# david-cortes/MatrixExtra

Hardware: AMD Instinct MI355X
Metric: CSR x dense SpMM GFLOP/s (fp64, 1M x 100k, 32 nnz/row, k=128) + achieved HBM BW% vs CPU ref (higher is better)
Workload: dtype f64; 1 GPU; dgRMatrix 1000000x100000 nnz/row=32 f64 %*% dense 100000x128 (BASELINE configs[1]); C col-major; rows_per_gpu=1000000, cols=100000, nnz_per_row=32, dense_cols=128, parallelism=single

## Files before the change

### matrixextra_amd/csrc/spmm_common.h

```cpp
#pragma once
#include "mx_dispatch.h"

struct mx_spmm_plan {
    int m = 0, K = 0, npanels = 0, panel_cols = 0, noct = 0;
    long long total_steps = 0;
    long long nnz = 0;
    int32_t *step_off = nullptr; size_t step_off_cap = 0;
    int32_t *pcol = nullptr;     size_t pcol_cap = 0;
    double *pval = nullptr;      size_t pval_cap = 0;
    void *scratch = nullptr;     size_t scratch_cap = 0;
    bool ready = false;
    bool pending = false;
    const int32_t *indptr = nullptr, *indices = nullptr;
    const double *values = nullptr;
    const int32_t *oct_off = nullptr;
    const long long *sizes = nullptr;
    int *go = nullptr;
    long long fill_cap = 0;
    int pad_rule = 0;
};

namespace mx {

template <typename T, int N> struct VecT;
template <> struct VecT<double, 1> { using type = double; };
template <> struct VecT<double, 2> { using type = double __attribute__((ext_vector_type(2))); };
template <> struct VecT<float, 1>  { using type = float; };
template <> struct VecT<float, 2>  { using type = float __attribute__((ext_vector_type(2))); };
template <> struct VecT<float, 4>  { using type = float __attribute__((ext_vector_type(4))); };

template <typename real_t, int VEC>
__device__ __forceinline__ void vload(real_t (&dst)[VEC], const real_t *__restrict__ p)
{
    using V = typename VecT<real_t, VEC>::type;
    if constexpr (VEC == 1) {
        dst[0] = *p;
    } else {
        const V v = *reinterpret_cast<const V *>(p);
#pragma unroll
        for (int i = 0; i < VEC; i++) dst[i] = v[i];
    }
}

template <typename real_t, int VEC>
__device__ __forceinline__ void vstore(real_t *__restrict__ p, const real_t (&src)[VEC])
{
    using V = typename VecT<real_t, VEC>::type;
    if constexpr (VEC == 1) {
        *p = src[0];
    } else {
        V v;
#pragma unroll
        for (int i = 0; i < VEC; i++) v[i] = src[i];
        *reinterpret_cast<V *>(p) = v;
    }
}

template <typename real_t, int VEC>
__device__ __forceinline__ void vstore_nt(real_t *__restrict__ p, const real_t (&src)[VEC])
{
    using V = typename VecT<real_t, VEC>::type;
    if constexpr (VEC == 1) {
        __builtin_nontemporal_store(src[0], p);
    } else {
        V v;
#pragma unroll
        for (int i = 0; i < VEC; i++) v[i] = src[i];
        __builtin_nontemporal_store(v, reinterpret_cast<V *>(p));
    }
}

__device__ __forceinline__ double mx_fma(double a, double b, double c) { return __builtin_fma(a, b, c); }
__device__ __forceinline__ float mx_fma(float a, float b, float c) { return __builtin_fmaf(a, b, c); }

constexpr int SLAB_GROUP = 8;
template <typename real_t> constexpr int SLAB_VEC = 16 / (int)sizeof(real_t);
template <typename real_t> constexpr int SLAB_W = SLAB_GROUP * SLAB_VEC<real_t>;

__device__ __forceinline__ void xcd_timing_barrier(unsigned *ctr, unsigned target)
{
    __syncthreads();
    if (threadIdx.x == 0) {
        __hip_atomic_fetch_add(ctr, 1u, __ATOMIC_RELAXED, __HIP_MEMORY_SCOPE_AGENT);
        int spins = 0;
        while (__hip_atomic_load(ctr, __ATOMIC_RELAXED, __HIP_MEMORY_SCOPE_AGENT) < target && ++spins < 4096)
            __builtin_amdgcn_s_sleep(8);
    }
    __syncthreads();
}

inline int pick_panels(int K, size_t l2_budget)
{
    const size_t slab_bytes = (size_t)K * 128;
    int p = (int)((slab_bytes + l2_budget - 1) / l2_budget);
    if (p < 1) p = 1;
    if (p > 64) p = 64;
    return p;
}

template <typename real_t>
inline bool slab_ok(int n, const real_t *B, size_t ldb, const real_t *C, size_t ldc, int colmajor)
{
    constexpr int VEC = SLAB_VEC<real_t>;
    if (n < VEC || n % VEC || ldb % VEC || (uintptr_t)B % 16) return false;
    if (!colmajor && (ldc % VEC || (uintptr_t)C % 16)) return false;
    return true;
}

#pragma GCC visibility push(hidden)
void kt_begin(hipStream_t st);
void kt_end(hipStream_t st);
void note_spmm_kernel(const char *name);
unsigned persistent_grid(int wg_per_cu, long long total_items);
constexpr size_t SYNC_BYTES = 8 * 64 * sizeof(unsigned);
void *pack_workspace(size_t bytes);
unsigned *sync_workspace();

template <typename real_t>
int launch_repack(int K, int Kp, int n, const real_t *B, size_t ldb, real_t *Bp, const int *go, hipStream_t st);
int launch_spmm_slab(int m, int n, int K, const int32_t *indptr, const int32_t *indices, const double *values,
                     const void *B, size_t ldb, void *C, size_t ldc, int dense_dtype, int colmajor, int npanels,
                     int wg_per_cu, hipStream_t stream);

int plan_begin(mx_spmm_plan *pl, int m, int K, const int32_t *indptr, const int32_t *indices, const double *values,
               int npanels, hipStream_t st, int pad_rule = 0);
int plan_end(mx_spmm_plan *pl, hipStream_t st, bool *refilled = nullptr);
int plan_repack(int K, int n, const void *B, size_t ldb, int dense_dtype, hipStream_t st, void **Bp_out,
                const int *go = nullptr);
int plan_run(const mx_spmm_plan *pl, int n, const void *B, size_t ldb, void *C, size_t ldc, int dense_dtype,
             int colmajor, int wg_per_cu, int sync_mode, hipStream_t st, const void *Bp = nullptr);
#pragma GCC visibility pop

}
```

### matrixextra_amd/csrc/spmm_plan.hip

```cpp
#include "spmm_common.h"
#include <new>

namespace mx {

constexpr int PLAN_RB = 8;
constexpr int PLAN_OCT_ROWS = PLAN_RB * 8;
constexpr int PLAN_MAXP = 64;
constexpr int PLAN_DEFAULT_WG_PER_CU = 1;
constexpr int PLAN_CHUNK = 4;
constexpr int PLAN_TAIL_SLOTS = 512;
constexpr int PLAN_ROW_SHIFT = 27;

constexpr int PLAN_LD = 4;
constexpr int PLAN_STAGE_STEPS = 384;
constexpr int PLAN_PAD_NUM = 7, PLAN_PAD_DEN = 4;

__host__ __device__ __forceinline__ bool plan_accept(long long total, long long nnz, long long cap_slots, int pad_rule)
{
    if (total < 0 || total * 8 + PLAN_TAIL_SLOTS > cap_slots) return false;
    return !(pad_rule && total * 8 * PLAN_PAD_DEN > nnz * PLAN_PAD_NUM + 65536LL * PLAN_PAD_DEN);
}

__device__ __forceinline__ int panel_of(int col, int panel_cols, float inv_pc, int npanels)
{
    int q = (int)((float)col * inv_pc);
    const int r = col - q * panel_cols;
    q += r >= panel_cols ? 1 : (r < 0 ? -1 : 0);
    return q < npanels ? q : npanels - 1;
}

__global__ __launch_bounds__(256)
void plan_size_kernel(int m, int noct, const int32_t *__restrict__ indptr, int32_t *__restrict__ steps,
                      long long *__restrict__ nnz_out)
{
    const int b = blockIdx.x * 256 + threadIdx.x;
    if (b == 0) *nnz_out = indptr[m];
    int len = 0;
    if (b < noct * 8) {
        const int r0 = min(b * PLAN_RB, m), r1 = min(b * PLAN_RB + PLAN_RB, m);
        len = indptr[r1] - indptr[r0];
    }
    len = max(len, __shfl_xor(len, 1, 8));
    len = max(len, __shfl_xor(len, 2, 8));
    len = max(len, __shfl_xor(len, 4, 8));
    if (b < noct * 8 && (b & 7) == 0)
        steps[b >> 3] = (len + 8 * PLAN_CHUNK - 1) & ~(8 * PLAN_CHUNK - 1);
}

__device__ __forceinline__ unsigned long long multisplit_peers(int key, const unsigned long long (&bal)[6], int nbits,
                                                                unsigned long long valid)
{
    unsigned long long peers = valid;
#pragma unroll
    for (int b = 0; b < 6; b++)
        if (b < nbits) peers &= ((key >> b) & 1) ? bal[b] : ~bal[b];
    return peers;
}

__global__ __launch_bounds__(512, 8)
void plan_fill_kernel(int m, int npanels, int panel_cols, const int32_t *__restrict__ indptr,
                      const int32_t *__restrict__ indices, const double *__restrict__ values,
                      const int32_t *__restrict__ oct_off, int32_t *__restrict__ pcol, double *__restrict__ pval,
                      int noct, int pad_col, int32_t *__restrict__ step_off,
                      const long long *__restrict__ sizes, long long cap_slots, int pad_rule, int *__restrict__ go)
{
    __shared__ int32_t s_col[PLAN_STAGE_STEPS * 8];
    __shared__ double s_val[PLAN_STAGE_STEPS * 8];
    __shared__ int s_bpo[8][PLAN_MAXP];

    const bool ok = plan_accept(sizes[0], sizes[1], cap_slots, pad_rule);
    if (blockIdx.x == 0 && threadIdx.x == 0) *go = ok ? 1 : 0;
    if (!ok) return;

    const int g = threadIdx.x >> 6, lane = threadIdx.x & 63;
    const int oct = blockIdx.x;
    const int row0 = oct * PLAN_OCT_ROWS + g * PLAN_RB;
    int rp[PLAN_RB + 1];
#pragma unroll
    for (int r = 0; r <= PLAN_RB; r++) rp[r] = uniform(indptr[min(row0 + r, m)]);
    const int s = rp[0], e = rp[PLAN_RB];
    const int base = oct_off[oct];
    const int steps_oct = oct_off[oct + 1] - base;
    const bool stage = steps_oct <= PLAN_STAGE_STEPS;
    const float inv_pc = 1.0f / (float)panel_cols;
    const int nbits = npanels > 1 ? 32 - __clz(npanels - 1) : 0;
    const unsigned long long below = (1ULL << lane) - 1ULL;

    int col0[PLAN_LD];
    double val0[PLAN_LD];
#pragma unroll
    for (int c = 0; c < PLAN_LD; c++) {
        const int k = s + 64 * c + lane;
        col0[c] = -1; val0[c] = 0.0;
        if (k < e) { col0[c] = indices[k]; val0[c] = values[k]; }
    }
    auto split = [&](int pan, unsigned long long (&bal)[6]) -> unsigned long long {
#pragma unroll
        for (int b = 0; b < 6; b++)
            bal[b] = b < nbits ? __ballot(pan >= 0 && ((pan >> b) & 1)) : 0ULL;
        return __ballot(pan >= 0);
    };

    int mine = 0;
    for (int k0 = s; k0 < e; k0 += 64 * PLAN_LD) {
        int colv[PLAN_LD];
#pragma unroll
        for (int c = 0; c < PLAN_LD; c++) {
            const int k = k0 + 64 * c + lane;
            colv[c] = col0[c];
            if (k0 != s) colv[c] = k < e ? indices[k] : -1;
        }
#pragma unroll
        for (int c = 0; c < PLAN_LD; c++) {
            if (k0 + 64 * c >= e) break;
            const int pan = colv[c] >= 0 ? panel_of(colv[c], panel_cols, inv_pc, npanels) : -1;
            unsigned long long bal[6];
            const unsigned long long valid = split(pan, bal);
            if (lane < npanels) mine += __popcll(multisplit_peers(lane, bal, nbits, valid));
        }
    }
    int incl = lane < npanels ? mine : 0;
#pragma unroll
    for (int off = 1; off < 64; off <<= 1) {
        const int up = __shfl_up(incl, off, 64);
        if (lane >= off) incl += up;
    }
    int nextstep = incl - mine;
    s_bpo[g][lane] = nextstep;

    auto put = [&](int t, int word, double v) {
        const int slot = (t & ~7) * 8 + g * 8 + (t & 7);
        if (stage) { s_col[slot] = word; s_val[slot] = v; }
        else { pcol[(size_t)base * 8 + slot] = word; pval[(size_t)base * 8 + slot] = v; }
    };

    for (int k0 = s; k0 < e; k0 += 64 * PLAN_LD) {
        int colv[PLAN_LD];
        double av[PLAN_LD];
#pragma unroll
        for (int c = 0; c < PLAN_LD; c++) {
            const int k = k0 + 64 * c + lane;
            colv[c] = col0[c]; av[c] = val0[c];
            if (k0 != s) {
                colv[c] = -1; av[c] = 0.0;
                if (k < e) { colv[c] = indices[k]; av[c] = values[k]; }
            }
        }
#pragma unroll
        for (int c = 0; c < PLAN_LD; c++) {
            if (k0 + 64 * c >= e) break;
            const int k = k0 + 64 * c + lane;
            const int col = colv[c];
            int pan = -1, lrow = 0;
            if (col >= 0) {
                pan = panel_of(col, panel_cols, inv_pc, npanels);
#pragma unroll
                for (int r = 1; r < PLAN_RB; r++) lrow += k >= rp[r];
            }
            unsigned long long bal[6];
            const unsigned long long valid = split(pan, bal);
            const int start = __shfl(nextstep, pan < 0 ? 0 : pan, 64);
            if (pan >= 0) put(start + __popcll(multisplit_peers(pan, bal, nbits, valid) & below), col | (lrow << PLAN_ROW_SHIFT), av[c]);
            if (lane < npanels) nextstep += __popcll(multisplit_peers(lane, bal, nbits, valid));
        }
    }
    int last_lrow = 0;
    if (e > s) {
#pragma unroll
        for (int r = 1; r < PLAN_RB; r++) last_lrow += (e - 1) >= rp[r];
    }
    for (int t = (e - s) + lane; t < steps_oct; t += 64) put(t, pad_col | (last_lrow << PLAN_ROW_SHIFT), 0.0);

    __syncthreads();
    if (g == 0 && lane < npanels) {
        int sum = 0;
#pragma unroll
        for (int gg = 0; gg < 8; gg++) sum += s_bpo[gg][lane];
        step_off[(size_t)oct * npanels + lane] = base + (lane == 0 ? 0 : sum / 8);
        if (oct == noct - 1 && lane == 0) step_off[(size_t)noct * npanels] = oct_off[noct];
    }
    if (stage) {
        const int nslots = steps_oct * 8;
        int4 *gc = reinterpret_cast<int4 *>(pcol + (size_t)base * 8);
        const int4 *lc = reinterpret_cast<const int4 *>(s_col);
        for (int i = threadIdx.x; i < nslots / 4; i += 512) gc[i] = lc[i];
        using d2 = double __attribute__((ext_vector_type(2)));
        d2 *gv = reinterpret_cast<d2 *>(pval + (size_t)base * 8);
        const d2 *lv = reinterpret_cast<const d2 *>(s_val);
        for (int i = threadIdx.x; i < nslots / 2; i += 512) gv[i] = lv[i];
    }
    if (oct == noct - 1) {
        static_assert(PLAN_TAIL_SLOTS == 512, "one slot per thread of the last block");
        const size_t dst = (size_t)oct_off[noct] * 8 + threadIdx.x;
        pcol[dst] = pad_col;
        pval[dst] = 0.0;
    }
}

template <int U>
__device__ __forceinline__ int group8_dpp_bcast(int v)
{
    int t = __builtin_amdgcn_mov_dpp(v, 0x150 + U, 0xF, 0x3, false);
    return __builtin_amdgcn_update_dpp(t, v, 0x150 + 8 + U, 0xF, 0xC, false);
}
template <int U>
__device__ __forceinline__ void plan_bcast(int pcw, double pvw, int &pc, double &pv)
{
    union { double d; int i[2]; } a, b;
    a.d = pvw;
    pc = group8_dpp_bcast<U>(pcw);
    b.i[0] = group8_dpp_bcast<U>(a.i[0]);
    b.i[1] = group8_dpp_bcast<U>(a.i[1]);
    pv = b.d;
}

template <int VEC>
__device__ __forceinline__ void lds_fold(double *d, double (&acc)[VEC])
{
#pragma unroll
    for (int v = 0; v < VEC; v++) __hip_atomic_fetch_add(d + v, acc[v], __ATOMIC_RELAXED, __HIP_MEMORY_SCOPE_WORKGROUP);
}
template <int VEC>
__device__ __forceinline__ void lds_fold(float *d, float (&acc)[VEC])
{
#pragma unroll
    for (int v = 0; v < VEC; v++) d[v] += acc[v];
}

#ifdef MX_SWEEP_PROBE
__device__ unsigned long long g_sweep_probe[8][8];
#define MX_PROBE(...) __VA_ARGS__
#else
#define MX_PROBE(...)
#endif

template <typename real_t, bool COLMAJOR, int PLAN_WAVES>
__global__ __launch_bounds__(PLAN_WAVES * 64)
void spmm_plan_kernel(int m, int n, int npanels, const int32_t *__restrict__ step_off,
                      const int32_t *__restrict__ pcol, const double *__restrict__ pval,
                      const real_t *__restrict__ Bp, size_t slab_stride,
                      real_t *__restrict__ C, size_t ldc, int nslabs, int ngens, int noct, int pad_col,
                      unsigned *__restrict__ sync_ctr, int sync_mode)
{
    constexpr int VEC = 16 / (int)sizeof(real_t);
    constexpr int W = SLAB_GROUP * VEC;
    constexpr int U = 8;
    constexpr int PLAN_WG_ROWS = PLAN_OCT_ROWS * PLAN_WAVES;
    constexpr int S = W + 16 / (int)sizeof(real_t) / 2;
    __shared__ real_t accs[PLAN_WG_ROWS * S];

    const int lane = threadIdx.x & 63, wave = threadIdx.x >> 6, g = lane >> 3, lg = lane & 7;
    const int xcd = blockIdx.x & 7, wg = blockIdx.x >> 3, nwg = gridDim.x >> 3;
    const long long total = (long long)nslabs * ngens;
    const long long lo = total * xcd / 8, hi = total * (xcd + 1) / 8;
    const int niter = (int)((hi - lo + nwg - 1) / nwg);
    unsigned *const my_ctr = sync_ctr + xcd * 64;
    real_t *const my_oct = accs + (size_t)wave * PLAN_OCT_ROWS * S;
    real_t *const my_rows = my_oct + (size_t)g * PLAN_RB * S + lg * VEC;
    MX_PROBE(long long pr_t = 0; int pr_kind = 0; unsigned long long pr_sum[3] = {0, 0, 0}; unsigned pr_cnt[3] = {0, 0, 0};)

    for (int it = 0; it < niter; it++) {
        const long long item_raw = lo + wg + (long long)it * nwg;
        const bool have = item_raw < hi;
        const long long item = have ? item_raw : lo;
        const int slab = (int)(item / ngens), gen = (int)(item % ngens);
        const int oct = gen * PLAN_WAVES + wave;
        const bool oct_ok = have && oct < noct;
        const char *__restrict__ Bbase = reinterpret_cast<const char *>(Bp + (size_t)slab * slab_stride);
        const unsigned lane_off = (unsigned)(lg * VEC * sizeof(real_t));

        for (int i = lane; i < PLAN_OCT_ROWS * S; i += 64) my_oct[i] = 0;
        if (sync_mode > 0) __syncthreads();

        {
            if (sync_mode >= 2) xcd_timing_barrier(my_ctr, (unsigned)(it + 1) * (unsigned)nwg);
            int so_row = 0, so_end = 0;
            if (oct_ok) {
                if (lane < npanels) so_row = step_off[(size_t)oct * npanels + lane];
                so_end = step_off[(size_t)oct * npanels + npanels];
            }
            const int sbeg = __builtin_amdgcn_readfirstlane(so_row);
            const int send = __builtin_amdgcn_readfirstlane(so_end);
            int next_b = npanels > 1 ? __builtin_amdgcn_readlane(so_row, 1) : send;
            int p = 0;
            int cur = 0;
            real_t acc[VEC];
#pragma unroll
            for (int v = 0; v < VEC; v++) acc[v] = 0;
            static_assert(U == 8, "one batch = one wavefront of plan slots");
            static_assert(W * sizeof(real_t) == 128, "slab line");
            auto b_offset = [&](int c) -> unsigned {
                return ((unsigned)c * (unsigned)(W * sizeof(real_t))) + lane_off;
            };
            int rc[PLAN_CHUNK], rn[PLAN_CHUNK];
            double rv[PLAN_CHUNK], rvn[PLAN_CHUNK];
            auto load_chunk = [&](int step, int (&c)[PLAN_CHUNK], double (&v)[PLAN_CHUNK]) {
                const long long e = (long long)step * 8 + lane;
#pragma unroll
                for (int k = 0; k < PLAN_CHUNK; k++) { c[k] = pcol[e + 64 * k]; v[k] = pval[e + 64 * k]; }
            };
            int pc[U];
            double pv[U];
            real_t b[U][VEC];
#pragma unroll
            for (int u = 0; u < U; u++) {
                pc[u] = 0;
                pv[u] = 0.0;
#pragma unroll
                for (int v = 0; v < VEC; v++) b[u][v] = 0;
            }
            auto consume = [&](int u) {
                const int lrow = (int)((unsigned)pc[u] >> PLAN_ROW_SHIFT);
                if (lrow != cur) {
                    lds_fold<VEC>(my_rows + cur * S, acc);
#pragma unroll
                    for (int v = 0; v < VEC; v++) acc[v] = 0;
                    cur = lrow;
                }
                const real_t a = (real_t)pv[u];
#pragma unroll
                for (int v = 0; v < VEC; v++) acc[v] = mx_fma(a, b[u][v], acc[v]);
#pragma unroll
                for (int v = 0; v < VEC; v++) asm volatile("" : "+v"(acc[v]));
                __builtin_amdgcn_sched_barrier(0);
            };
            if (send > sbeg) {
                load_chunk(sbeg, rc, rv);
#pragma unroll
                for (int k = 0; k < PLAN_CHUNK; k++) asm volatile("" : "+v"(rc[k]), "+v"(rv[k]));
            }
            for (int s = sbeg; s < send; s += U * PLAN_CHUNK) {
                load_chunk(s + U * PLAN_CHUNK, rn, rvn);
                __builtin_amdgcn_sched_barrier(0);
#pragma unroll
                for (int k = 0; k < PLAN_CHUNK; k++) {
#define MX_PLAN_STEP(UU)                                                                                              \
                    consume(UU);                                                                                      \
                    plan_bcast<UU>(rc[k], rv[k], pc[UU], pv[UU]);                                                     \
                    vload<real_t, VEC>(b[UU], reinterpret_cast<const real_t *>(Bbase + b_offset(pc[UU])));            \
                    __builtin_amdgcn_sched_barrier(0);
                    MX_PLAN_STEP(0)
                    MX_PROBE(if (pr_kind && !(pr_kind == 3 && s == sbeg && k == 0)) {
                        const unsigned long long dt = (unsigned long long)(wall_clock64() - pr_t);
                        _Pragma("unroll") for (int j = 0; j < 3; j++)
                            if (pr_kind == j + 1) { pr_sum[j] += dt; pr_cnt[j]++; }
                        pr_kind = 0;
                    })
                    MX_PLAN_STEP(1) MX_PLAN_STEP(2) MX_PLAN_STEP(3)
                    MX_PLAN_STEP(4) MX_PLAN_STEP(5) MX_PLAN_STEP(6) MX_PLAN_STEP(7)
#undef MX_PLAN_STEP
                    MX_PROBE(bool pr_met = false;)
                    if (sync_mode > 0) {
                        const int sn = s + U * k;
                        while (p < npanels - 1 && sn >= next_b) {
                            p++;
                            __syncthreads();
                            MX_PROBE(pr_met = true; if (pr_kind != 3) pr_t = wall_clock64();)
                            next_b = p < npanels - 1 ? __builtin_amdgcn_readlane(so_row, p + 1) : send;
                        }
                    }
                    MX_PROBE(if (pr_kind != 3) { pr_kind = pr_met ? 2 : 1; if (!pr_met) pr_t = wall_clock64(); })
                }
#pragma unroll
                for (int k = 0; k < PLAN_CHUNK; k++) { rc[k] = rn[k]; rv[k] = rvn[k]; }
            }
            MX_PROBE(if (send > sbeg) { pr_kind = 3; pr_t = wall_clock64(); })
#pragma unroll
            for (int u = 0; u < U; u++) consume(u);
            lds_fold<VEC>(my_rows + cur * S, acc);
            if (sync_mode > 0)
                for (; p < npanels - 1; p++) __syncthreads();
        }

        if (oct_ok) {
            const int row_base = gen * PLAN_WG_ROWS + wave * PLAN_OCT_ROWS;
            const int ncols = min(W, n - slab * W);
            if constexpr (!COLMAJOR) {
#pragma unroll
                for (int rr = 0; rr < PLAN_OCT_ROWS / 8; rr++) {
                    const int r = rr * 8 + g;
                    const int row = row_base + r;
                    if (row < m && lg * VEC < ncols) {
                        real_t t[VEC];
#pragma unroll
                        for (int v = 0; v < VEC; v++) t[v] = my_oct[(size_t)r * S + lg * VEC + v];
                        vstore_nt<real_t, VEC>(C + (size_t)row * ldc + slab * W + lg * VEC, t);
                    }
                }
            } else {
                const int row = row_base + lane;
                if (row < m) {
                    for (int c = 0; c < ncols; c++)
                        __builtin_nontemporal_store(my_oct[(size_t)lane * S + c], &C[(size_t)(slab * W + c) * ldc + row]);
                }
            }
        }
    }
    MX_PROBE(if (lane == 0) {
        for (int j = 0; j < 3; j++) {
            atomicAdd(&g_sweep_probe[xcd][2 * j], pr_sum[j]);
            atomicAdd(&g_sweep_probe[xcd][2 * j + 1], (unsigned long long)pr_cnt[j]);
        }
        atomicAdd(&g_sweep_probe[xcd][6], 1ULL);
    })
}

static int grow(void **p, size_t *cap, size_t bytes)
{
    if (*cap >= bytes && *p) return 0;
    if (*p) (void)hipFree(*p);
    *p = nullptr; *cap = 0;
    MX_HIP(hipMalloc(p, bytes ? bytes : 16));
    *cap = bytes;
    return 0;
}

struct PlanReadback {
    long long *host = nullptr;
    hipEvent_t ev = nullptr;
};
static PlanReadback *plan_readback()
{
    static thread_local PlanReadback rb;
    if (!rb.host) {
        if (hipHostMalloc((void **)&rb.host, 2 * sizeof(long long), hipHostMallocDefault) != hipSuccess) { rb.host = nullptr; return nullptr; }
        if (hipEventCreateWithFlags(&rb.ev, hipEventDisableTiming) != hipSuccess) { (void)hipHostFree(rb.host); rb.host = nullptr; return nullptr; }
    }
    return &rb;
}

int plan_begin(mx_spmm_plan *pl, int m, int K, const int32_t *indptr, const int32_t *indices, const double *values,
               int npanels, hipStream_t st, int pad_rule)
{
    pl->ready = false;
    pl->pending = false;
    MX_REQUIRE(K < (1 << 25), "spmm plan: more than 2^25 columns (32-bit slab offsets)");
    if (npanels <= 0) npanels = pick_panels(K, (size_t)1600 << 10);
    if (npanels > PLAN_MAXP) npanels = PLAN_MAXP;
    pl->m = m; pl->K = K; pl->npanels = npanels;
    pl->panel_cols = (int)ceil_div(K > 0 ? K : 1, npanels);
    pl->noct = (int)ceil_div(m, PLAN_OCT_ROWS);
    pl->total_steps = 0; pl->nnz = 0;
    if (m == 0) { pl->ready = true; return 0; }
    const size_t nop = (size_t)pl->noct * npanels;
    const size_t al = 255;
    const size_t steps_b = (((size_t)pl->noct * 4) + al) & ~al;
    const size_t octoff_b = ((((size_t)pl->noct + 1) * 4) + al) & ~al;
    const size_t rb_b = 256;
    if (grow(&pl->scratch, &pl->scratch_cap, steps_b + octoff_b + rb_b + scan_workspace_bytes((int64_t)pl->noct))) return 1;
    if (grow((void **)&pl->step_off, &pl->step_off_cap, (nop + 1) * 4)) return 1;
    int32_t *steps = (int32_t *)pl->scratch;
    int32_t *oct_off = (int32_t *)((char *)steps + steps_b);
    long long *rb_dev = (long long *)((char *)oct_off + octoff_b);
    void *scan_ws = (char *)rb_dev + rb_b;
    const unsigned sblocks = (unsigned)ceil_div((long long)pl->noct * 8, 256);
    hipLaunchKernelGGL(plan_size_kernel, dim3(sblocks), dim3(256), 0, st, m, pl->noct, indptr, steps, rb_dev + 1);
    MX_LAUNCH_CHECK();
    if (exclusive_scan_i32(steps, (int64_t)pl->noct, oct_off, (int64_t *)rb_dev, scan_ws, st)) return 1;
    PlanReadback *rb = plan_readback();
    MX_REQUIRE(rb, "spmm plan: cannot allocate the pinned read-back buffer");
    MX_HIP(hipMemcpyAsync(rb->host, rb_dev, 2 * sizeof(long long), hipMemcpyDeviceToHost, st));
    MX_HIP(hipEventRecord(rb->ev, st));
    pl->indptr = indptr; pl->indices = indices; pl->values = values;
    pl->oct_off = oct_off; pl->sizes = rb_dev; pl->go = (int *)(rb_dev + 2);
    pl->pad_rule = pad_rule;
    pl->fill_cap = (long long)std::min(pl->pcol_cap / 4, pl->pval_cap / 8);
    hipLaunchKernelGGL(plan_fill_kernel, dim3((unsigned)pl->noct), dim3(512), 0, st, m, npanels, pl->panel_cols, indptr,
                       indices, values, oct_off, pl->pcol, pl->pval, pl->noct, K, pl->step_off, pl->sizes, pl->fill_cap,
                       pad_rule, pl->go);
    MX_LAUNCH_CHECK();
    pl->pending = true;
    return 0;
}

int plan_end(mx_spmm_plan *pl, hipStream_t st, bool *refilled)
{
    if (refilled) *refilled = false;
    if (!pl->pending) return 0;
    pl->pending = false;
    PlanReadback *rb = plan_readback();
    MX_HIP(hipEventSynchronize(rb->ev));
    const long long total = rb->host[0];
    pl->nnz = (int32_t)rb->host[1];
    MX_REQUIRE(total >= 0 && total * 8 <= (long long)INT_MAX * 4LL, "spmm plan: too many steps (%lld)", total);
    MX_REQUIRE(total <= (long long)INT_MAX, "spmm plan: step offsets exceed int32");
    pl->total_steps = total;
    if (plan_accept(total, pl->nnz, pl->fill_cap, pl->pad_rule)) { pl->ready = true; return 0; }
    if (plan_accept(total, pl->nnz, LLONG_MAX, pl->pad_rule) == false) return 0;
    const size_t slots = (size_t)total * 8 + PLAN_TAIL_SLOTS;
    if (grow((void **)&pl->pcol, &pl->pcol_cap, slots * 4)) return 1;
    if (grow((void **)&pl->pval, &pl->pval_cap, slots * 8)) return 1;
    pl->fill_cap = (long long)std::min(pl->pcol_cap / 4, pl->pval_cap / 8);
    hipLaunchKernelGGL(plan_fill_kernel, dim3((unsigned)pl->noct), dim3(512), 0, st, pl->m, pl->npanels, pl->panel_cols,
                       pl->indptr, pl->indices, pl->values, pl->oct_off, pl->pcol, pl->pval, pl->noct, pl->K, pl->step_off,
                       pl->sizes, pl->fill_cap, pl->pad_rule, pl->go);
    MX_LAUNCH_CHECK();
    pl->ready = true;
    if (refilled) *refilled = true;
    return 0;
}

int plan_repack(int K, int n, const void *B, size_t ldb, int dense_dtype, hipStream_t st, void **Bp_out, const int *go)
{
    return dispatch_dense("spmm plan", dense_dtype, [&](auto t) {
        using real_t = typename decltype(t)::type;
        constexpr int W = SLAB_W<real_t>;
        const int nslabs = (int)ceil_div(n, W), Kp = K + 1;
        real_t *Bp = (real_t *)pack_workspace((size_t)nslabs * (size_t)Kp * W * sizeof(real_t));
        MX_REQUIRE(Bp, "spmm plan: cannot allocate the packed copy of B");
        if (launch_repack<real_t>(K, Kp, n, (const real_t *)B, ldb, Bp, go, st)) return 1;
        *Bp_out = Bp;
        return 0;
    });
}

int plan_run(const mx_spmm_plan *pl, int n, const void *B, size_t ldb, void *C, size_t ldc, int dense_dtype,
             int colmajor, int wg_per_cu, int sync_mode, hipStream_t st, const void *Bp)
{
    const char *what = "mxd_spmm_plan_run";
    return dispatch_dense(what, dense_dtype, [&](auto t) {
        using real_t = typename decltype(t)::type;
        constexpr int W = SLAB_W<real_t>;
        MX_REQUIRE(slab_ok<real_t>(n, (const real_t *)B, ldb, (const real_t *)C, ldc, colmajor),
                   "mxd_spmm_plan_run: operands do not meet the 16-byte alignment rules");
        const int m = pl->m, K = pl->K;
        const int nslabs = (int)ceil_div(n, W);
        if (!Bp) {
            void *packed = nullptr;
            if (plan_repack(K, n, B, ldb, dense_dtype, st, &packed)) return 1;
            Bp = packed;
        }
        if (wg_per_cu != 1 && wg_per_cu != 2 && wg_per_cu != 4) wg_per_cu = PLAN_DEFAULT_WG_PER_CU;
        const int waves = 16 / wg_per_cu;
        const int ngens = (int)ceil_div(m, PLAN_OCT_ROWS * waves);
        const unsigned grid = persistent_grid(wg_per_cu, (long long)nslabs * ngens);
        unsigned *sync = sync_workspace();
        if (!sync || pl->npanels <= 1) sync_mode = 0;
        if (sync_mode >= 2) MX_HIP(hipMemsetAsync(sync, 0, SYNC_BYTES, st));
        return dispatch_int(int_list<16, 8, 4>{}, what, "wavefronts per workgroup", waves, [&](auto wv) {
            return dispatch_int(int_list<0, 1>{}, what, "colmajor", colmajor ? 1 : 0, [&](auto cm) {
                kt_begin(st);
                hipLaunchKernelGGL((spmm_plan_kernel<real_t, cm() != 0, wv()>), dim3(grid), dim3(wv() * 64), 0, st, m, n,
                                   pl->npanels, pl->step_off, pl->pcol, pl->pval, (const real_t *)Bp, (size_t)(K + 1) * W,
                                   (real_t *)C, ldc, nslabs, ngens, pl->noct, K, sync, sync_mode);
                kt_end(st);
                MX_LAUNCH_CHECK();
                return 0;
            });
        });
    });
}

}

extern "C" int mxd_spmm_plan_create(int m, int K, const int32_t *indptr, const int32_t *indices, const double *values,
                                    int npanels, void *stream, mx_spmm_plan **plan_out)
{
    MX_REQUIRE(plan_out && m >= 0 && K >= 0, "mxd_spmm_plan_create: bad arguments");
    mx_spmm_plan *pl = *plan_out ? *plan_out : new (std::nothrow) mx_spmm_plan();
    MX_REQUIRE(pl, "out of host memory");
    const hipStream_t st = mx::as_stream(stream);
    if (mx::plan_begin(pl, m, K, indptr, indices, values, npanels, st) || mx::plan_end(pl, st)) {
        if (!*plan_out) { mxd_spmm_plan_destroy(pl); }
        return 1;
    }
    *plan_out = pl;
    return 0;
}

extern "C" int mxd_spmm_plan_destroy(mx_spmm_plan *pl)
{
    if (!pl) return 0;
    if (pl->step_off) (void)hipFree(pl->step_off);
    if (pl->pcol) (void)hipFree(pl->pcol);
    if (pl->pval) (void)hipFree(pl->pval);
    if (pl->scratch) (void)hipFree(pl->scratch);
    delete pl;
    return 0;
}

extern "C" int mxd_spmm_plan_info(const mx_spmm_plan *pl, int *npanels, int64_t *padded_entries)
{
    MX_REQUIRE(pl, "mxd_spmm_plan_info: null plan");
    if (npanels) *npanels = pl->npanels;
    if (padded_entries) *padded_entries = pl->total_steps * 8;
    return 0;
}

extern "C" int mxd_spmm_plan_copy_to_host(const mx_spmm_plan *pl, int32_t *step_off, int32_t *pcol, double *pval,
                                          void *stream)
{
    MX_REQUIRE(pl && step_off && pcol && pval, "mxd_spmm_plan_copy_to_host: null pointer");
    MX_REQUIRE(pl->ready, "mxd_spmm_plan_copy_to_host: the plan was sized but not built");
    if (pl->m == 0) return 0;
    const hipStream_t st = mx::as_stream(stream);
    const size_t nso = (size_t)pl->noct * pl->npanels + 1;
    const size_t slots = (size_t)pl->total_steps * 8 + mx::PLAN_TAIL_SLOTS;
    MX_HIP(hipMemcpyAsync(step_off, pl->step_off, nso * sizeof(int32_t), hipMemcpyDeviceToHost, st));
    MX_HIP(hipMemcpyAsync(pcol, pl->pcol, slots * sizeof(int32_t), hipMemcpyDeviceToHost, st));
    MX_HIP(hipMemcpyAsync(pval, pl->pval, slots * sizeof(double), hipMemcpyDeviceToHost, st));
    MX_HIP(hipStreamSynchronize(st));
    return 0;
}

extern "C" int mxd_spmm_plan_run(const mx_spmm_plan *pl, int n, const void *B, size_t ldb, void *C, size_t ldc,
                                 int dense_dtype, int colmajor_out, int wg_per_cu, int sync_mode, void *stream)
{
    MX_REQUIRE(pl && n >= 0, "mxd_spmm_plan_run: bad arguments");
    MX_REQUIRE(pl->ready, "mxd_spmm_plan_run: the plan was sized but not built");
    if (pl->m == 0 || n == 0) return 0;
    MX_REQUIRE(B && C, "mxd_spmm_plan_run: null pointer");
    hipStream_t st = mx::as_stream(stream);
    if (sync_mode < 0) sync_mode = 1;
    mx::note_spmm_kernel("spmm_plan_kernel");
    return mx::plan_run(pl, n, B, ldb, C, ldc, dense_dtype, colmajor_out, wg_per_cu, sync_mode, st);
}

#ifdef MX_SWEEP_PROBE
extern "C" int mxd_spmm_sweep_probe(unsigned long long *out64)
{
    static const unsigned long long zeros[64] = {};
    MX_HIP(hipDeviceSynchronize());
    MX_HIP(hipMemcpyFromSymbol(out64, HIP_SYMBOL(mx::g_sweep_probe), sizeof(zeros)));
    MX_HIP(hipMemcpyToSymbol(HIP_SYMBOL(mx::g_sweep_probe), zeros, sizeof(zeros)));
    return 0;
}
#endif
```

Baseline: 3960 GFLOP/s.

## Replace plan exclusive scan with tile sums and in-kernel prefix; template fill on panel bits

Removes the separate exclusive-scan pass over per-octet step counts. The size kernel now also emits per-tile partial sums, and each fill block rebuilds its own offset by summing earlier tile sums plus the steps inside its own tile. The fill kernel is templated on the number of panel bits. It classifies the first chunk once and reuses the rank and count in the scatter pass, instead of redoing the ballots. This trades a kernel launch and a scan pass for redundant per-block reductions, and the total steps are now summed on the host from the read-back tile sums.

```diff
diff --git a/matrixextra_amd/csrc/spmm_common.h b/matrixextra_amd/csrc/spmm_common.h
--- a/matrixextra_amd/csrc/spmm_common.h
+++ b/matrixextra_amd/csrc/spmm_common.h
@@ -13,8 +13,10 @@
     bool pending = false;
     const int32_t *indptr = nullptr, *indices = nullptr;
     const double *values = nullptr;
-    const int32_t *oct_off = nullptr;
-    const long long *sizes = nullptr;
+    const int32_t *steps = nullptr;
+    const unsigned *tile_sums = nullptr;
+    int ntiles = 0, tile_octs = 0;
+    const long long *nnz_dev = nullptr;
     int *go = nullptr;
     long long fill_cap = 0;
     int pad_rule = 0;
diff --git a/matrixextra_amd/csrc/spmm_plan.hip b/matrixextra_amd/csrc/spmm_plan.hip
--- a/matrixextra_amd/csrc/spmm_plan.hip
+++ b/matrixextra_amd/csrc/spmm_plan.hip
@@ -14,6 +14,10 @@
 constexpr int PLAN_LD = 4;
 constexpr int PLAN_STAGE_STEPS = 384;
 constexpr int PLAN_PAD_NUM = 7, PLAN_PAD_DEN = 4;
+constexpr int PLAN_MAX_TILES = 4096;
+constexpr int PLAN_RB_HEAD = 16;
+
+inline int plan_tile_octs(int noct) { return 32 * (int)ceil_div(noct > 0 ? noct : 1, 32 * PLAN_MAX_TILES); }
 
 __host__ __device__ __forceinline__ bool plan_accept(long long total, long long nnz, long long cap_slots, int pad_rule)
 {
@@ -30,61 +34,106 @@
 }
 
 __global__ __launch_bounds__(256)
-void plan_size_kernel(int m, int noct, const int32_t *__restrict__ indptr, int32_t *__restrict__ steps,
-                      long long *__restrict__ nnz_out)
-{
-    const int b = blockIdx.x * 256 + threadIdx.x;
-    if (b == 0) *nnz_out = indptr[m];
-    int len = 0;
-    if (b < noct * 8) {
-        const int r0 = min(b * PLAN_RB, m), r1 = min(b * PLAN_RB + PLAN_RB, m);
-        len = indptr[r1] - indptr[r0];
-    }
-    len = max(len, __shfl_xor(len, 1, 8));
-    len = max(len, __shfl_xor(len, 2, 8));
-    len = max(len, __shfl_xor(len, 4, 8));
-    if (b < noct * 8 && (b & 7) == 0)
-        steps[b >> 3] = (len + 8 * PLAN_CHUNK - 1) & ~(8 * PLAN_CHUNK - 1);
-}
-
-__device__ __forceinline__ unsigned long long multisplit_peers(int key, const unsigned long long (&bal)[6], int nbits,
+void plan_size_kernel(int m, int noct, int tile_octs, const int32_t *__restrict__ indptr, int32_t *__restrict__ steps,
+                      unsigned *__restrict__ tile_sums, long long *__restrict__ nnz_out)
+{
+    __shared__ unsigned s_part[4];
+    if (blockIdx.x == 0 && threadIdx.x == 0) *nnz_out = indptr[m];
+    unsigned sum = 0;
+    for (int o = 0; o < tile_octs; o += 32) {
+        const long long bl = ((long long)blockIdx.x * tile_octs + o) * 8 + threadIdx.x;
+        const bool live = bl < (long long)noct * 8;
+        const int b = live ? (int)bl : 0;
+        int len = 0;
+        if (live) {
+            const int r0 = (int)min((long long)b * PLAN_RB, (long long)m), r1 = (int)min((long long)b * PLAN_RB + PLAN_RB, (long long)m);
+            len = indptr[r1] - indptr[r0];
+        }
+        len = max(len, __shfl_xor(len, 1, 8));
+        len = max(len, __shfl_xor(len, 2, 8));
+        len = max(len, __shfl_xor(len, 4, 8));
+        if (live && (b & 7) == 0) {
+            const int st = (len + 8 * PLAN_CHUNK - 1) & ~(8 * PLAN_CHUNK - 1);
+            steps[b >> 3] = st;
+            sum += (unsigned)st;
+        }
+    }
+#pragma unroll
+    for (int off = 32; off > 0; off >>= 1) sum += __shfl_xor(sum, off, 64);
+    if ((threadIdx.x & 63) == 0) s_part[threadIdx.x >> 6] = sum;
+    __syncthreads();
+    if (threadIdx.x == 0) tile_sums[blockIdx.x] = s_part[0] + s_part[1] + s_part[2] + s_part[3];
+}
+
+__device__ __forceinline__ int wave_sum(int v)
+{
+    v += __builtin_amdgcn_update_dpp(0, v, 0xB1, 0xF, 0xF, true);
+    v += __builtin_amdgcn_update_dpp(0, v, 0x4E, 0xF, 0xF, true);
+    v += __builtin_amdgcn_update_dpp(0, v, 0x141, 0xF, 0xF, true);
+    v += __builtin_amdgcn_update_dpp(0, v, 0x140, 0xF, 0xF, true);
+    return __builtin_amdgcn_readlane(v, 0) + __builtin_amdgcn_readlane(v, 16) + __builtin_amdgcn_readlane(v, 32) +
+           __builtin_amdgcn_readlane(v, 48);
+}
+
+template <int NBITS>
+__device__ __forceinline__ unsigned long long multisplit_peers(int key, const unsigned long long (&bal)[6],
                                                                 unsigned long long valid)
 {
     unsigned long long peers = valid;
 #pragma unroll
-    for (int b = 0; b < 6; b++)
-        if (b < nbits) peers &= ((key >> b) & 1) ? bal[b] : ~bal[b];
+    for (int b = 0; b < NBITS; b++) peers &= ((key >> b) & 1) ? bal[b] : ~bal[b];
     return peers;
 }
 
+template <int NBITS>
 __global__ __launch_bounds__(512, 8)
 void plan_fill_kernel(int m, int npanels, int panel_cols, const int32_t *__restrict__ indptr,
                       const int32_t *__restrict__ indices, const double *__restrict__ values,
-                      const int32_t *__restrict__ oct_off, int32_t *__restrict__ pcol, double *__restrict__ pval,
+                      const int32_t *__restrict__ steps, const unsigned *__restrict__ tile_sums, int ntiles, int tile_octs,
+                      int32_t *__restrict__ pcol, double *__restrict__ pval,
                       int noct, int pad_col, int32_t *__restrict__ step_off,
-                      const long long *__restrict__ sizes, long long cap_slots, int pad_rule, int *__restrict__ go)
+                      const long long *__restrict__ nnz_dev, long long cap_slots, int pad_rule, int *__restrict__ go)
 {
     __shared__ int32_t s_col[PLAN_STAGE_STEPS * 8];
     __shared__ double s_val[PLAN_STAGE_STEPS * 8];
     __shared__ int s_bpo[8][PLAN_MAXP];
-
-    const bool ok = plan_accept(sizes[0], sizes[1], cap_slots, pad_rule);
+    __shared__ long long s_tot[8];
+    __shared__ int s_front[8];
+
+    const int g = threadIdx.x >> 6, lane = threadIdx.x & 63;
+    const int oct = blockIdx.x;
+
+    const int tile = oct / tile_octs, oct0 = tile * tile_octs;
+    int part_lo = 0, part_hi = 0, part_front = 0;
+    for (int i = threadIdx.x; i < ntiles; i += 512) {
+        const unsigned v = tile_sums[i];
+        part_lo += (int)(v & 0xffffu);
+        part_hi += (int)(v >> 16);
+        part_front += i < tile ? (int)v : 0;
+    }
+    for (int i = oct0 + threadIdx.x; i < oct; i += 512) part_front += steps[i];
+    const int steps_oct = steps[oct];
+    const long long nnz = *nnz_dev;
+
+    const int row0 = oct * PLAN_OCT_ROWS + g * PLAN_RB;
+    int rp[PLAN_RB + 1];
+#pragma unroll
+    for (int r = 0; r <= PLAN_RB; r++) rp[r] = uniform(indptr[min(row0 + r, m)]);
+    const int s = rp[0], e = rp[PLAN_RB];
+    const bool stage = steps_oct <= PLAN_STAGE_STEPS;
+    const float inv_pc = 1.0f / (float)panel_cols;
+
+    const int wave_lo = wave_sum(part_lo), wave_hi = wave_sum(part_hi), wave_front = wave_sum(part_front);
+    if (lane == 0) { s_tot[g] = ((long long)wave_hi << 16) + wave_lo; s_front[g] = wave_front; }
+    __syncthreads();
+    long long total = 0;
+    int base = 0;
+#pragma unroll
+    for (int w = 0; w < 8; w++) { total += s_tot[w]; base += s_front[w]; }
+
+    const bool ok = plan_accept(total, nnz, cap_slots, pad_rule);
     if (blockIdx.x == 0 && threadIdx.x == 0) *go = ok ? 1 : 0;
     if (!ok) return;
-
-    const int g = threadIdx.x >> 6, lane = threadIdx.x & 63;
-    const int oct = blockIdx.x;
-    const int row0 = oct * PLAN_OCT_ROWS + g * PLAN_RB;
-    int rp[PLAN_RB + 1];
-#pragma unroll
-    for (int r = 0; r <= PLAN_RB; r++) rp[r] = uniform(indptr[min(row0 + r, m)]);
-    const int s = rp[0], e = rp[PLAN_RB];
-    const int base = oct_off[oct];
-    const int steps_oct = oct_off[oct + 1] - base;
-    const bool stage = steps_oct <= PLAN_STAGE_STEPS;
-    const float inv_pc = 1.0f / (float)panel_cols;
-    const int nbits = npanels > 1 ? 32 - __clz(npanels - 1) : 0;
-    const unsigned long long below = (1ULL << lane) - 1ULL;
 
     int col0[PLAN_LD];
     double val0[PLAN_LD];
@@ -94,34 +143,43 @@
         col0[c] = -1; val0[c] = 0.0;
         if (k < e) { col0[c] = indices[k]; val0[c] = values[k]; }
     }
+
     auto split = [&](int pan, unsigned long long (&bal)[6]) -> unsigned long long {
 #pragma unroll
-        for (int b = 0; b < 6; b++)
-            bal[b] = b < nbits ? __ballot(pan >= 0 && ((pan >> b) & 1)) : 0ULL;
+        for (int b = 0; b < NBITS; b++) bal[b] = __ballot(pan >= 0 && ((pan >> b) & 1));
         return __ballot(pan >= 0);
     };
-
+    auto classify = [&](int pan, int &rank, int &cnt) {
+        unsigned long long bal[6];
+        const unsigned long long valid = split(pan, bal);
+        const unsigned long long peers = multisplit_peers<NBITS>(pan, bal, valid);
+        rank = __builtin_amdgcn_mbcnt_hi((unsigned)(peers >> 32), __builtin_amdgcn_mbcnt_lo((unsigned)peers, 0u));
+        cnt = lane < npanels ? __popcll(multisplit_peers<NBITS>(lane, bal, valid)) : 0;
+    };
+
+    int cls0[PLAN_LD];
     int mine = 0;
-    for (int k0 = s; k0 < e; k0 += 64 * PLAN_LD) {
-        int colv[PLAN_LD];
-#pragma unroll
-        for (int c = 0; c < PLAN_LD; c++) {
-            const int k = k0 + 64 * c + lane;
-            colv[c] = col0[c];
-            if (k0 != s) colv[c] = k < e ? indices[k] : -1;
-        }
-#pragma unroll
-        for (int c = 0; c < PLAN_LD; c++) {
-            if (k0 + 64 * c >= e) break;
-            const int pan = colv[c] >= 0 ? panel_of(colv[c], panel_cols, inv_pc, npanels) : -1;
-            unsigned long long bal[6];
-            const unsigned long long valid = split(pan, bal);
-            if (lane < npanels) mine += __popcll(multisplit_peers(lane, bal, nbits, valid));
-        }
-    }
-    int incl = lane < npanels ? mine : 0;
-#pragma unroll
-    for (int off = 1; off < 64; off <<= 1) {
+#pragma unroll
+    for (int c = 0; c < PLAN_LD; c++) {
+        cls0[c] = 0xff;
+        if (s + 64 * c < e) {
+            const int pan = col0[c] >= 0 ? panel_of(col0[c], panel_cols, inv_pc, npanels) : -1;
+            int rank, cnt;
+            classify(pan, rank, cnt);
+            cls0[c] = (pan & 0xff) | (rank << 8) | (cnt << 16);
+            mine += cnt;
+        }
+    }
+    for (int k0 = s + 64 * PLAN_LD; k0 < e; k0 += 64) {
+        const int k = k0 + lane;
+        const int pan = k < e ? panel_of(indices[k], panel_cols, inv_pc, npanels) : -1;
+        int rank, cnt;
+        classify(pan, rank, cnt);
+        mine += cnt;
+    }
+    int incl = mine;
+#pragma unroll
+    for (int off = 1; off < (1 << NBITS); off <<= 1) {
         const int up = __shfl_up(incl, off, 64);
         if (lane >= off) incl += up;
     }
@@ -133,42 +191,35 @@
         if (stage) { s_col[slot] = word; s_val[slot] = v; }
         else { pcol[(size_t)base * 8 + slot] = word; pval[(size_t)base * 8 + slot] = v; }
     };
-
-    for (int k0 = s; k0 < e; k0 += 64 * PLAN_LD) {
-        int colv[PLAN_LD];
-        double av[PLAN_LD];
-#pragma unroll
-        for (int c = 0; c < PLAN_LD; c++) {
-            const int k = k0 + 64 * c + lane;
-            colv[c] = col0[c]; av[c] = val0[c];
-            if (k0 != s) {
-                colv[c] = -1; av[c] = 0.0;
-                if (k < e) { colv[c] = indices[k]; av[c] = values[k]; }
-            }
-        }
-#pragma unroll
-        for (int c = 0; c < PLAN_LD; c++) {
-            if (k0 + 64 * c >= e) break;
-            const int k = k0 + 64 * c + lane;
-            const int col = colv[c];
-            int pan = -1, lrow = 0;
-            if (col >= 0) {
-                pan = panel_of(col, panel_cols, inv_pc, npanels);
-#pragma unroll
-                for (int r = 1; r < PLAN_RB; r++) lrow += k >= rp[r];
-            }
-            unsigned long long bal[6];
-            const unsigned long long valid = split(pan, bal);
+    auto local_row = [&](int k) {
+        int lrow = 0;
+#pragma unroll
+        for (int r = 1; r < PLAN_RB; r++) lrow += k >= rp[r];
+        return lrow;
+    };
+
+#pragma unroll
+    for (int c = 0; c < PLAN_LD; c++) {
+        if (s + 64 * c < e) {
+            const int pan = (int)(signed char)cls0[c], rank = (cls0[c] >> 8) & 0xff, cnt = cls0[c] >> 16;
             const int start = __shfl(nextstep, pan < 0 ? 0 : pan, 64);
-            if (pan >= 0) put(start + __popcll(multisplit_peers(pan, bal, nbits, valid) & below), col | (lrow << PLAN_ROW_SHIFT), av[c]);
-            if (lane < npanels) nextstep += __popcll(multisplit_peers(lane, bal, nbits, valid));
-        }
-    }
-    int last_lrow = 0;
-    if (e > s) {
-#pragma unroll
-        for (int r = 1; r < PLAN_RB; r++) last_lrow += (e - 1) >= rp[r];
-    }
+            if (pan >= 0) put(start + rank, col0[c] | (local_row(s + 64 * c + lane) << PLAN_ROW_SHIFT), val0[c]);
+            nextstep += cnt;
+        }
+    }
+    for (int k0 = s + 64 * PLAN_LD; k0 < e; k0 += 64) {
+        const int k = k0 + lane;
+        int col = -1;
+        double av = 0.0;
+        if (k < e) { col = indices[k]; av = values[k]; }
+        const int pan = col >= 0 ? panel_of(col, panel_cols, inv_pc, npanels) : -1;
+        int rank, cnt;
+        classify(pan, rank, cnt);
+        const int start = __shfl(nextstep, pan < 0 ? 0 : pan, 64);
+        if (pan >= 0) put(start + rank, col | (local_row(k) << PLAN_ROW_SHIFT), av);
+        nextstep += cnt;
+    }
+    const int last_lrow = e > s ? local_row(e - 1) : 0;
     for (int t = (e - s) + lane; t < steps_oct; t += 64) put(t, pad_col | (last_lrow << PLAN_ROW_SHIFT), 0.0);
 
     __syncthreads();
@@ -177,7 +228,7 @@
 #pragma unroll
         for (int gg = 0; gg < 8; gg++) sum += s_bpo[gg][lane];
         step_off[(size_t)oct * npanels + lane] = base + (lane == 0 ? 0 : sum / 8);
-        if (oct == noct - 1 && lane == 0) step_off[(size_t)noct * npanels] = oct_off[noct];
+        if (oct == noct - 1 && lane == 0) step_off[(size_t)noct * npanels] = (int32_t)total;
     }
     if (stage) {
         const int nslots = steps_oct * 8;
@@ -191,7 +242,7 @@
     }
     if (oct == noct - 1) {
         static_assert(PLAN_TAIL_SLOTS == 512, "one slot per thread of the last block");
-        const size_t dst = (size_t)oct_off[noct] * 8 + threadIdx.x;
+        const size_t dst = (size_t)total * 8 + threadIdx.x;
         pcol[dst] = pad_col;
         pval[dst] = 0.0;
     }
@@ -416,17 +467,31 @@
 }
 
 struct PlanReadback {
-    long long *host = nullptr;
+    char *host = nullptr;
     hipEvent_t ev = nullptr;
 };
+constexpr size_t PLAN_RB_BYTES = PLAN_RB_HEAD + PLAN_MAX_TILES * sizeof(unsigned);
 static PlanReadback *plan_readback()
 {
     static thread_local PlanReadback rb;
     if (!rb.host) {
-        if (hipHostMalloc((void **)&rb.host, 2 * sizeof(long long), hipHostMallocDefault) != hipSuccess) { rb.host = nullptr; return nullptr; }
+        if (hipHostMalloc((void **)&rb.host, PLAN_RB_BYTES, hipHostMallocDefault) != hipSuccess) { rb.host = nullptr; return nullptr; }
         if (hipEventCreateWithFlags(&rb.ev, hipEventDisableTiming) != hipSuccess) { (void)hipHostFree(rb.host); rb.host = nullptr; return nullptr; }
     }
     return &rb;
+}
+
+static int launch_fill(const mx_spmm_plan *pl, hipStream_t st)
+{
+    const int nbits = pl->npanels > 1 ? 32 - __builtin_clz((unsigned)(pl->npanels - 1)) : 0;
+    return dispatch_int(int_list<0, 1, 2, 3, 4, 5, 6>{}, "spmm plan", "panel bits", nbits, [&](auto nb) {
+        hipLaunchKernelGGL((plan_fill_kernel<nb()>), dim3((unsigned)pl->noct), dim3(512), 0, st, pl->m, pl->npanels,
+                           pl->panel_cols, pl->indptr, pl->indices, pl->values, pl->steps, pl->tile_sums, pl->ntiles,
+                           pl->tile_octs, pl->pcol, pl->pval, pl->noct, pl->K, pl->step_off, pl->nnz_dev, pl->fill_cap,
+                           pl->pad_rule, pl->go);
+        MX_LAUNCH_CHECK();
+        return 0;
+    });
 }
 
 int plan_begin(mx_spmm_plan *pl, int m, int K, const int32_t *indptr, const int32_t *indices, const double *values,
@@ -445,30 +510,26 @@
     const size_t nop = (size_t)pl->noct * npanels;
     const size_t al = 255;
     const size_t steps_b = (((size_t)pl->noct * 4) + al) & ~al;
-    const size_t octoff_b = ((((size_t)pl->noct + 1) * 4) + al) & ~al;
-    const size_t rb_b = 256;
-    if (grow(&pl->scratch, &pl->scratch_cap, steps_b + octoff_b + rb_b + scan_workspace_bytes((int64_t)pl->noct))) return 1;
+    pl->tile_octs = plan_tile_octs(pl->noct);
+    pl->ntiles = (int)ceil_div(pl->noct, pl->tile_octs);
+    if (grow(&pl->scratch, &pl->scratch_cap, steps_b + PLAN_RB_BYTES)) return 1;
     if (grow((void **)&pl->step_off, &pl->step_off_cap, (nop + 1) * 4)) return 1;
     int32_t *steps = (int32_t *)pl->scratch;
-    int32_t *oct_off = (int32_t *)((char *)steps + steps_b);
-    long long *rb_dev = (long long *)((char *)oct_off + octoff_b);
-    void *scan_ws = (char *)rb_dev + rb_b;
-    const unsigned sblocks = (unsigned)ceil_div((long long)pl->noct * 8, 256);
-    hipLaunchKernelGGL(plan_size_kernel, dim3(sblocks), dim3(256), 0, st, m, pl->noct, indptr, steps, rb_dev + 1);
+    char *rb_dev = (char *)steps + steps_b;
+    pl->steps = steps;
+    pl->nnz_dev = (long long *)rb_dev; pl->go = (int *)(rb_dev + 8);
+    pl->tile_sums = (unsigned *)(rb_dev + PLAN_RB_HEAD);
+    hipLaunchKernelGGL(plan_size_kernel, dim3((unsigned)pl->ntiles), dim3(256), 0, st, m, pl->noct, pl->tile_octs, indptr,
+                       steps, (unsigned *)(rb_dev + PLAN_RB_HEAD), (long long *)rb_dev);
     MX_LAUNCH_CHECK();
-    if (exclusive_scan_i32(steps, (int64_t)pl->noct, oct_off, (int64_t *)rb_dev, scan_ws, st)) return 1;
     PlanReadback *rb = plan_readback();
     MX_REQUIRE(rb, "spmm plan: cannot allocate the pinned read-back buffer");
-    MX_HIP(hipMemcpyAsync(rb->host, rb_dev, 2 * sizeof(long long), hipMemcpyDeviceToHost, st));
+    MX_HIP(hipMemcpyAsync(rb->host, rb_dev, PLAN_RB_HEAD + (size_t)pl->ntiles * sizeof(unsigned), hipMemcpyDeviceToHost, st));
     MX_HIP(hipEventRecord(rb->ev, st));
     pl->indptr = indptr; pl->indices = indices; pl->values = values;
-    pl->oct_off = oct_off; pl->sizes = rb_dev; pl->go = (int *)(rb_dev + 2);
     pl->pad_rule = pad_rule;
     pl->fill_cap = (long long)std::min(pl->pcol_cap / 4, pl->pval_cap / 8);
-    hipLaunchKernelGGL(plan_fill_kernel, dim3((unsigned)pl->noct), dim3(512), 0, st, m, npanels, pl->panel_cols, indptr,
-                       indices, values, oct_off, pl->pcol, pl->pval, pl->noct, K, pl->step_off, pl->sizes, pl->fill_cap,
-                       pad_rule, pl->go);
-    MX_LAUNCH_CHECK();
+    if (launch_fill(pl, st)) return 1;
     pl->pending = true;
     return 0;
 }
@@ -480,8 +541,11 @@
     pl->pending = false;
     PlanReadback *rb = plan_readback();
     MX_HIP(hipEventSynchronize(rb->ev));
-    const long long total = rb->host[0];
-    pl->nnz = (int32_t)rb->host[1];
+    const long long nnz = *(const long long *)rb->host;
+    long long total = 0;
+    const unsigned *sums = (const unsigned *)(rb->host + PLAN_RB_HEAD);
+    for (int i = 0; i < pl->ntiles; i++) total += sums[i];
+    pl->nnz = (int32_t)nnz;
     MX_REQUIRE(total >= 0 && total * 8 <= (long long)INT_MAX * 4LL, "spmm plan: too many steps (%lld)", total);
     MX_REQUIRE(total <= (long long)INT_MAX, "spmm plan: step offsets exceed int32");
     pl->total_steps = total;
@@ -491,10 +555,7 @@
     if (grow((void **)&pl->pcol, &pl->pcol_cap, slots * 4)) return 1;
     if (grow((void **)&pl->pval, &pl->pval_cap, slots * 8)) return 1;
     pl->fill_cap = (long long)std::min(pl->pcol_cap / 4, pl->pval_cap / 8);
-    hipLaunchKernelGGL(plan_fill_kernel, dim3((unsigned)pl->noct), dim3(512), 0, st, pl->m, pl->npanels, pl->panel_cols,
-                       pl->indptr, pl->indices, pl->values, pl->oct_off, pl->pcol, pl->pval, pl->noct, pl->K, pl->step_off,
-                       pl->sizes, pl->fill_cap, pl->pad_rule, pl->go);
-    MX_LAUNCH_CHECK();
+    if (launch_fill(pl, st)) return 1;
     pl->ready = true;
     if (refilled) *refilled = true;
     return 0;
```

Measured after the change: 4044 GFLOP/s (median of 6 runs). +2.1%, better.
